# krishnanlab/PecanPy

Hardware: AMD Instinct MI355X
Metric: million walk-steps/sec on RMAT-22 SparseOTF p=0.5 q=2 (higher is better)
Workload: dtype f32

## Files before the change

include/pecanpy_amd.h:

```cpp
#ifndef PECANPY_AMD_H
#define PECANPY_AMD_H

#include <stdint.h>

#ifdef __cplusplus
extern "C" {
#endif

typedef struct pw_graph pw_graph;

typedef enum {
    PW_OK = 0,
    PW_ERR_INVALID = -1,
    PW_ERR_HIP = -2,
    PW_ERR_NO_DEVICE = -3,
    PW_ERR_UNSUPPORTED = -4,
    PW_ERR_NOMEM = -5
} pw_status;

typedef enum {
    PW_MODE_SPARSE_OTF = 0,
    PW_MODE_DENSE_OTF = 1,
    PW_MODE_PRECOMP = 2,
    PW_MODE_FIRST_ORDER_UNWEIGHTED = 3,
// ... 281 lines not shown
int pw_selftest_seqscan_f64(const double *x, uint32_t n, double r, int use_target, uint32_t chunk,
                            uint32_t *index, double *sum);

int pw_selftest_exact_decision(const uint8_t *cls, uint32_t n, float w_out, float w_prev, const double *r,
                               uint32_t n_r, uint32_t *chain, uint32_t *exact);
int pw_selftest_lane(int on_device, int device, const uint8_t *cls, uint32_t n, float w_out, float w_prev, const double *r,
                     uint32_t n_r, uint32_t *chain, uint32_t *lane, uint32_t *kmax, uint32_t *tight, uint32_t *chain_lane);
int pw_selftest_lane_floats(int on_device, int device, const uint8_t *cls, uint32_t n, float w_out, float w_prev,
                            const double *r, uint32_t n_r, uint32_t *chain, uint32_t *lane, float *tots);
int pw_selftest_lane_unit_bounded(const uint8_t *cls, uint32_t n, float w_out, float w_prev, const double *r, uint32_t n_r,
                                  uint32_t *chain, uint32_t *lane);
int pw_selftest_lane_unit_tight(const uint8_t *cls, uint32_t n, float w_out, float w_prev, const double *r, uint32_t n_r,
                                uint32_t *chain, uint32_t *lane, uint32_t *tight);
int pw_selftest_lane_weighted(const float *vals, const float *base, const uint8_t *cls, uint32_t n, const double *r,
                              uint32_t n_r, uint32_t *chain, uint32_t *lane);
int pw_selftest_exact_decision_f64(const uint8_t *cls, uint32_t n, double w_out, double w_prev, const double *r,
                                   uint32_t n_r, uint32_t *chain, uint32_t *exact);

#ifdef __cplusplus
}
#endif
#endif
```

pecanpy_amd/_lib.py:

```python
import ctypes as C
import os
import subprocess

_HERE = os.path.dirname(os.path.abspath(__file__))
LIB_PATH = os.environ.get("PECANPY_AMD_LIB") or os.path.join(_HERE, "libpecanpy_amd.so")
_lib = None


class PwStats(C.Structure):
    _fields_ = [
        ("total_steps", C.c_uint64),
        ("overflow_reads", C.c_uint64),
        ("clamped_reads", C.c_uint64),
        ("dead_end_walks", C.c_uint64),
        ("repair_rounds", C.c_uint64),
        ("walk_kernel_ms", C.c_double),
        ("rng_kernel_ms", C.c_double),
        ("walk_kernel_launches", C.c_uint32),
        ("stream_addressing", C.c_uint32),
        ("lane_kernel", C.c_uint32),
        ("lane_rounds", C.c_uint32),
        ("redo_walks", C.c_uint64),
        ("list_entries_read", C.c_uint64),
        ("ambiguous_steps", C.c_uint64),
# ... 310 lines not shown
    "pw_corpus_dev_shape": (C.c_int, [C.c_void_p] + [C.POINTER(C.c_uint64)] * 3),
    "pw_corpus_dev_fill": (C.c_int, [C.c_void_p, C.c_void_p]),
    "pw_corpus_dev_export": (C.c_int, [C.c_void_p, C.c_void_p]),
    "pw_corpus_dev_destroy": (None, [C.c_void_p]),
    "pw_selftest_edgelist_weight": (C.c_int, [C.c_char_p, C.c_uint64, _f64p]),
    "pw_selftest_edgelist_line": (C.c_int, [C.c_char_p, C.c_uint64, C.c_uint64, C.c_char_p, C.c_int, _u32p, C.c_void_p, _f64p]),
    "pw_selftest_exact_decision": (C.c_int, [C.c_void_p, C.c_uint32, C.c_float, C.c_float, C.c_void_p, C.c_uint32,
                                             C.c_void_p, C.c_void_p]),
    "pw_selftest_lane": (C.c_int, [C.c_int, C.c_int, C.c_void_p, C.c_uint32, C.c_float, C.c_float, C.c_void_p, C.c_uint32,
                                   C.c_void_p, C.c_void_p, C.c_void_p, C.c_void_p, C.c_void_p]),
    "pw_selftest_lane_floats": (C.c_int, [C.c_int, C.c_int, C.c_void_p, C.c_uint32, C.c_float, C.c_float, C.c_void_p, C.c_uint32,
                                          C.c_void_p, C.c_void_p, C.c_void_p]),
    "pw_selftest_lane_unit_bounded": (C.c_int, [C.c_void_p, C.c_uint32, C.c_float, C.c_float, C.c_void_p, C.c_uint32, C.c_void_p, C.c_void_p]),
    "pw_selftest_lane_unit_tight": (C.c_int, [C.c_void_p, C.c_uint32, C.c_float, C.c_float, C.c_void_p, C.c_uint32, C.c_void_p, C.c_void_p, C.c_void_p]),
    "pw_selftest_lane_weighted": (C.c_int, [C.c_void_p, C.c_void_p, C.c_void_p, C.c_uint32, C.c_void_p, C.c_uint32, C.c_void_p, C.c_void_p]),
    "pw_selftest_exact_decision_f64": (C.c_int, [C.c_void_p, C.c_uint32, C.c_double, C.c_double, C.c_void_p,
                                                 C.c_uint32, C.c_void_p, C.c_void_p]),
    "pw_selftest_seqscan_f32": (C.c_int, [C.c_void_p, C.c_uint32, C.c_double, C.c_int, C.c_uint32,
                                          _u32p, _f32p]),
    "pw_selftest_seqscan_f64": (C.c_int, [C.c_void_p, C.c_uint32, C.c_double, C.c_int, C.c_uint32,
                                          _u32p, _f64p]),
}


class PwError(RuntimeError):
    pass


def build(verbose=False):
    cmd = ["make", "-C", os.path.join(_HERE, "csrc")]
# ... 66 lines not shown
```

pecanpy_amd/csrc/pecanpy_amd.hip:

```cpp
#include <hip/hip_runtime.h>
#include <stdio.h>
#include <unistd.h>
#include <stdlib.h>
#include <string.h>

#include <new>
#include <random>
#include <algorithm>
#include <cerrno>
#include <chrono>
#include <condition_variable>
#include <functional>
#include <future>
#include <memory>
#include <mutex>
#include <cmath>
#include <string>
#include <thread>
#include <vector>

#include "../../include/pecanpy_amd.h"
#include "aux_kernels.hip.h"
#include "devmem.hpp"
#include "edgelist.hpp"
// ... 5030 lines not shown
        uint32_t kc = n;
        for (uint32_t k = 0; k < n; k++) {
            c = c + x[cls[k]];
            if (c >= r[i]) { kc = k; break; }
        }
        chain[i] = kc;
        const pw::ExactThresholds64 th = pw::exact_thresholds_f64(r[i] * S, (double)n, wmax);
        const uint32_t k1 = (uint32_t)(std::lower_bound(E.begin(), E.end(), th.lo) - E.begin());
        exact[i] = (k1 < n && E[k1] >= th.hi) ? k1 : 0xffffffffu;
    }
    return PW_OK;
}

namespace {

struct LaneRow {
    std::vector<uint16_t> cl16;
    std::vector<uint32_t> cl32;
    uint32_t n_cl = 0, pp = 0xffffffffu, wide = 0;
    uint32_t piv_off = 0;
    float tot = 0, x_in = 0, x_out = 0, x_prev = 0;
    pw::ListView view() const { return pw::list_view_of(wide ? (const void *)cl32.data() : (const void *)cl16.data(), wide, n_cl, piv_off); }
};

int lane_row_setup(const uint8_t *cls, uint32_t n, float w_out, float w_prev, LaneRow &row, bool need_pow2 = true) {
    auto pow2 = [](float w) { int e = 0; return std::frexp(w, &e) == 0.5f; };
    if (need_pow2 && (!pow2(w_out) || !pow2(w_prev))) return fail(PW_ERR_UNSUPPORTED, "biases must be powers of two");
    if (!(w_out > 0.0f) || !(w_prev > 0.0f)) return fail(PW_ERR_INVALID, "biases must be positive");
    uint32_t cnt[3] = {0, 0, 0};
    row.wide = n > 65536u ? 1u : 0u;
    for (uint32_t k = 0; k < n; k++) {
        if (cls[k] > 2) return fail(PW_ERR_INVALID, "class must be 0 (out), 1 (common) or 2 (prev)");
        cnt[cls[k]]++;
        if (cls[k] == 1) { if (row.wide) row.cl32.push_back(k); else row.cl16.push_back((uint16_t)k); }
        if (cls[k] == 2) row.pp = k;
    }
    if (cnt[2] > 1) return fail(PW_ERR_INVALID, "at most one prev");
    row.n_cl = cnt[1];
    row.cl16.resize(row.cl16.size() + 8, 0xffffu);
    row.cl32.resize(row.cl32.size() + 8, 0xffffffffu);
    if (pw::list_has_pivots(row.wide, row.n_cl) && !getenv("PW_SELFTEST_NO_PIVOTS")) {
        const uint32_t np = pw::list_pivot_count(row.wide), step = pw::list_pivot_step(row.wide, row.n_cl);
        row.piv_off = (uint32_t)(row.wide ? row.cl32.size() : row.cl16.size());
        for (uint32_t k = 0; k < np; k++) {
            if (row.wide) row.cl32.push_back(row.cl32[(size_t)(k + 1) * step]);
            else row.cl16.push_back(row.cl16[(size_t)(k + 1) * step]);
        }
    }
    row.tot = (float)((double)cnt[1] + (double)cnt[0] * (double)w_out + (double)cnt[2] * (double)w_prev);
    row.x_in = 1.0f / row.tot;
    row.x_out = row.x_in * w_out;
    row.x_prev = row.x_in * w_prev;
    return 0;
}

}

namespace pw {
PW_HD void lane_selftest_one(uint32_t n, const ListView &cl, uint32_t n_cl, uint32_t pp, float w_out, float w_prev, double r,
                             uint32_t *out) {
    LaneStep ls{0.0f, 0u, 0u, 0u, 0u, 0u, 0u};
    const uint32_t lane = lane_decide(n, n_cl, pp, r, w_out, w_prev, cl, ls);
// ... 277 lines not shown
            if (vals[k] < base[k]) any_neg = true;
            drun += (double)vals[k] - (double)base[k];
            dl.push_back(drun);
            if (wide) cl32.push_back(k); else cl16.push_back((uint16_t)k);
        } else if (cls[k] == 2) {
            if (pp != 0xffffffffu) return fail(PW_ERR_INVALID, "at most one prev");
            pp = k;
            dprev = (double)vals[k] - (double)base[k];
        } else if (cls[k] != 0 || vals[k] != base[k]) return fail(PW_ERR_INVALID, "class 0 elements carry their base value");
    }
    const uint32_t n_cl = (uint32_t)dl.size();
    cl16.resize(cl16.size() + 8, 0xffffu);
    cl32.resize(cl32.size() + 8, 0xffffffffu);
    uint32_t piv_off = 0;
    if (pw::list_has_pivots(wide, n_cl)) {
        const uint32_t np = pw::list_pivot_count(wide), step = pw::list_pivot_step(wide, n_cl);
        piv_off = (uint32_t)(wide ? cl32.size() : cl16.size());
        for (uint32_t k = 0; k < np; k++) { if (wide) cl32.push_back(cl32[(size_t)(k + 1) * step]); else cl16.push_back(cl16[(size_t)(k + 1) * step]); }
    }
    dl.push_back(0.0);
    const pw::ListView view = pw::list_view_of(wide ? (const void *)cl32.data() : (const void *)cl16.data(), wide, n_cl, piv_off);
    if (any_pos && any_neg) return fail(PW_ERR_INVALID, "the common neighbours' differences must share one sign (that of q - 1)");
    const pw::WeightedRow wr{pq.data(), dl.data(), dprev, !any_neg};
    for (uint32_t i = 0; i < n_r; i++) {
        uint32_t lo = 0, hi = n;
        while (lo < hi) { const uint32_t mid = (lo + hi) >> 1; if ((double)c[mid] >= r[i]) hi = mid; else lo = mid + 1; }
        chain[i] = lo;
        uint32_t probes = 0, k_safe = 0;
        lane[i] = pw::lane_decide_weighted(n, n_cl, pp, r[i], tot, wr, view, probes, k_safe);
        if (k_safe > chain[i]) return fail(PW_ERR_INVALID, "lane_decide_weighted: k_safe beyond the chain's position");
    }
    return PW_OK;
}

PW_EXPORT int pw_noise_thresholds_csr(const uint32_t *indptr, const float *data, uint32_t n_nodes, double gamma, float *thr) {
    if (!indptr || !thr || (!data && indptr[n_nodes] != 0)) return fail(PW_ERR_INVALID, "null pointer");
    pw::noise_thresholds_csr(indptr, data, n_nodes, gamma, thr);
    return PW_OK;
}

PW_EXPORT int pw_noise_thresholds_csr_numpy1(const uint32_t *indptr, const float *data, uint32_t n_nodes, double gamma, float *thr) {
    if (!indptr || !thr || (!data && indptr[n_nodes] != 0)) return fail(PW_ERR_INVALID, "null pointer");
    pw::noise_thresholds_csr(indptr, data, n_nodes, gamma, thr, true);
    return PW_OK;
}

PW_EXPORT int pw_noise_thresholds_csr_f64(const uint32_t *indptr, const float *data, uint32_t n_nodes, double gamma, float *thr) {
    if (!indptr || !thr) return fail(PW_ERR_INVALID, "null pointer");
    pw::noise_thresholds_csr_f64(indptr, data, n_nodes, gamma, thr);
// ... 76 lines not shown
```

pecanpy_amd/csrc/seqscan.h:

```cpp
#pragma once
#include <math.h>
#include <stdint.h>
#include <string.h>

#if defined(__HIPCC__)
#define PW_HD __host__ __device__ __forceinline__
#define PW_HD_CALL __host__ __device__ __attribute__((noinline))
#else
#define PW_HD inline
#define PW_HD_CALL inline
#endif

namespace pw {

template <typename T> struct FloatTraits;

template <> struct FloatTraits<float> {
    using UInt = uint32_t;
    static constexpr int MANT = 23;
    static constexpr int EXP_MASK = 0xff;
    static PW_HD UInt bits(float x) {
#if defined(__HIP_DEVICE_COMPILE__)
        return __float_as_uint(x);
#else
// ... 159 lines not shown
    if (prev_pos != 0xffffffffu && prev_pos >= s && k >= prev_pos) {
        const uint32_t need2 = need > wp ? need - wp : 0u;
        k = s + ((need2 + wo_m1) >> sh_out);
        if (k < prev_pos) k = prev_pos;
        e_k = base + ((k - s) << sh_out) + wp;
    }
    return k;
}

struct ListWin {
    uint32_t v[4];
};
constexpr uint32_t LIST_PIVOTS_NARROW = 20, LIST_PIVOTS_WIDE = 10;
PW_HD uint32_t list_pivot_count(uint32_t wide) { return wide ? LIST_PIVOTS_WIDE : LIST_PIVOTS_NARROW; }
PW_HD bool list_has_pivots(uint32_t wide, uint32_t n) { return n > list_pivot_count(wide); }
PW_HD uint32_t list_pivot_step(uint32_t wide, uint32_t n) { return wide ? n / (LIST_PIVOTS_WIDE + 1u) : n / (LIST_PIVOTS_NARROW + 1u); }

struct ListView {
    const void *p;
    uint32_t wide;
    const void *piv = nullptr;
    uint32_t npiv = 0;
    uint32_t step = 0;
    uint32_t tail = 0xffffffffu;
    uint32_t inl = 0;
    uint32_t tshift = 10;
#if defined(__HIP_DEVICE_COMPILE__)
    __device__ __forceinline__ uint32_t tail_entry(uint32_t i) const {
        const uint32_t o = 8u + (wide ? i << 2 : i << 1);
        const uint32_t addr = tail + ((o >> 4) << tshift) + (o & 15u);
        return wide ? *(const __attribute__((address_space(3))) uint32_t *)(uintptr_t)addr
                    : (uint32_t) * (const __attribute__((address_space(3))) uint16_t *)(uintptr_t)addr;
    }
#endif
    PW_HD uint32_t at(uint32_t i) const {
#if defined(__HIP_DEVICE_COMPILE__)
        if (tail != 0xffffffffu && inl) return tail_entry(i);
#endif
// ... 19 lines not shown
        }
#endif
        if (wide) {
            struct __attribute__((packed, aligned(4))) Raw { uint32_t v[4]; };
            const Raw raw = *(const Raw *)((const uint32_t *)p + w0);
            w.v[0] = raw.v[0]; w.v[1] = raw.v[1]; w.v[2] = raw.v[2]; w.v[3] = raw.v[3];
        } else {
            struct __attribute__((aligned(8))) Raw2 { uint32_t x, y; };
            const Raw2 raw = *(const Raw2 *)((const uint16_t *)p + w0);
            w.v[0] = raw.x & 0xffffu; w.v[1] = raw.x >> 16; w.v[2] = raw.y & 0xffffu; w.v[3] = raw.y >> 16;
        }
        return w;
    }
};

PW_HD ListView list_view_of(const void *cl, uint32_t wide, uint32_t n_cl, uint32_t piv_off) {
    ListView v{cl, wide};
    if (piv_off && list_has_pivots(wide, n_cl)) {
        v.piv = wide ? (const void *)((const uint32_t *)cl + piv_off) : (const void *)((const uint16_t *)cl + piv_off);
        v.npiv = list_pivot_count(wide);
        v.step = list_pivot_step(wide, n_cl);
    }
    return v;
}

PW_HD uint32_t list_lower_bound_pos(const ListView &cl, uint32_t n, uint32_t x) {
    uint32_t lo = 0, hi = n;
    if (cl.npiv) {
        uint32_t klo = 0, khi = cl.npiv;
        while (klo < khi) {
            const uint32_t km = (klo + khi) >> 1;
            if (cl.pivot(km) >= x) { khi = km; hi = (km + 1u) * cl.step; }
            else { klo = km + 1u; lo = (km + 1u) * cl.step + 1u; }
        }
    }
    while (lo < hi) {
        const uint32_t mid = (lo + hi) >> 1;
        if (cl.at(mid) < x) lo = mid + 1u; else hi = mid;
    }
    return lo;
}

PW_HD uint64_t div_floor_small(uint64_t a, uint64_t b) {
    uint64_t q = (uint64_t)((double)a / (double)b);
    if (q * b > a) q--;
    else if ((q + 1u) * b <= a) q++;
    return q;
}

struct SearchResult {
    uint32_t f;
    uint32_t p_below, p_at;
    uint64_t v_below, v_at;
    bool has_below;
};
template <class Eval>
PW_HD void list_search_pivots(const ListView &cl, const Eval &ev, uint64_t target, uint32_t &lo, uint32_t &hi, SearchResult &r) {
    uint32_t klo = 0, khi = cl.npiv;
    while (klo < khi) {
        const uint32_t km = (klo + khi) >> 1;
        const uint32_t ik = (km + 1u) * cl.step;
        if (ik < lo) { klo = km + 1u; continue; }
        const uint32_t P = cl.pivot(km);
        const uint64_t v = ev(ik, P);
        if (v >= target) { khi = km; hi = ik; r.p_at = P; r.v_at = v; }
        else { klo = km + 1u; lo = ik + 1u; r.p_below = P; r.v_below = v; r.has_below = true; }
    }
}

template <class Eval>
PW_HD SearchResult list_search(const ListView &cl, uint32_t lo_min, uint32_t n, const Eval &ev, uint64_t target, uint32_t &reads) {
    SearchResult r;
    r.p_below = 0; r.v_below = 0; r.has_below = false; r.p_at = 0xffffffffu; r.v_at = 0;
    uint32_t lo = lo_min, hi = n;
    if (cl.npiv) list_search_pivots(cl, ev, target, lo, hi, r);
    while (lo < hi) {
        const uint32_t mid = (lo + hi) >> 1;
        const uint32_t P = cl.at(mid);
        reads++;
        const uint64_t v = ev(mid, P);
        if (v >= target) { hi = mid; r.p_at = P; r.v_at = v; }
        else { lo = mid + 1u; r.p_below = P; r.v_below = v; r.has_below = true; }
    }
    r.f = lo;
    return r;
}

template <class Eval>
PW_HD SearchResult list_search_wide(const ListView &cl, uint32_t lo_min, uint32_t n, const Eval &ev, uint64_t target, uint32_t &reads) {
    SearchResult r;
    r.p_below = 0; r.v_below = 0; r.has_below = false; r.p_at = 0xffffffffu; r.v_at = 0;
    uint32_t lo = lo_min, hi = n;
    while (hi - lo >= 3u && hi > lo) {
        const uint32_t m2 = lo + ((hi - lo) >> 1);
        const uint32_t m1 = lo + ((m2 - lo) >> 1);
        const uint32_t m3 = m2 + 1u + ((hi - m2 - 1u) >> 1);
        const uint32_t P1 = cl.at(m1), P2 = cl.at(m2), P3 = cl.at(m3);
// ... 667 lines not shown
```

pecanpy_amd/csrc/walk_lanes.hip.h:

```cpp
#pragma once
#include "scan.hip.h"
#include "walk_sparse.hip.h"

namespace pw {

struct SuspRec {
    uint32_t job, j, s0, d;
    uint32_t n_in, pp, e, coff;
    uint32_t kmax, choice, soff_lo, soff_hi;
    float tot, wo;
    double r;
};
static_assert(sizeof(SuspRec) == 64, "queue record is four 16-byte accesses");

struct VerRec {
    uint32_t kmax, n_in, pp, choice;
    uint32_t e, coff, d, job;
    float tot, wo;
    double r;
};
static_assert(sizeof(VerRec) == 48, "verification record is three 16-byte stores");

constexpr uint32_t LANE_NEEDS_WAVE = 0xfffffff9u;
constexpr uint32_t LANE_EAGER_MARK = 0xffffffffu;
// ... 775 lines not shown
        } else {
            DecideCtx dc;
            SearchResult sr;
            sr.f = 0; sr.p_below = 0; sr.v_below = 0; sr.has_below = false; sr.p_at = 0xffffffffu; sr.v_at = 0;
            uint32_t s_lo = 0, s_hi = 0;
            bool need = false, go = false;
            const bool narrow = A.d <= 65536u;
            if (runnable && !nolist) {
                wo = A.j >= 2 ? w_out : 1.0f;
                choice = lane_decide_begin(A.d, A.n_in, A.pp, r, wo, w_prev, ls, dc);
                go = choice != LANE_REDO;
                if (go && A.n_in) {
                    const MassEval ev64{A.pp, dc.sh_in, dc.sh_out, dc.sh_prev};
                    const uint32_t wide = narrow ? 0u : 1u;
                    const bool inl = narrow && A.n_in <= EL_INLINE;
                    const uint32_t step = inl ? 1u : list_pivot_step(wide, A.n_in);
                    uint32_t klo = 0, khi = inl ? A.n_in : (list_has_pivots(wide, A.n_in) ? list_pivot_count(wide) : 0u);
                    s_hi = A.n_in;
                    while (klo < khi) {
                        const uint32_t km = (klo + khi) >> 1;
                        const uint32_t ik = inl ? km : (km + 1u) * step;
                        const uint32_t P = narrow ? q_u16(24u + (km << 1)) : q_u32(24u + (km << 2));
                        const uint32_t vm = (uint32_t)ev64(ik, P);
                        if (vm >= dc.lo_th) { khi = km; s_hi = ik; sr.p_at = P; sr.v_at = vm; }
                        else { klo = km + 1u; s_lo = ik + 1u; sr.p_below = P; sr.v_below = vm; sr.has_below = true; }
                    }
                    need = !inl && s_lo < s_hi;
                    sr.f = s_lo;
                }
            }
            for (uint32_t trip = 0; ballot(need); trip++) {
                const uint32_t esh = narrow ? 1u : 2u;
                const uint64_t lbase = (uint64_t)A.coff * 16u;
                uint32_t g = s_lo + ((s_hi - s_lo) >> 1);
                if (need && trip < 2u && sr.has_below && sr.p_at != 0xffffffffu && sr.v_at > sr.v_below) {
                    const float t = (float)(dc.lo_th - (uint32_t)sr.v_below) / (float)((uint32_t)sr.v_at - (uint32_t)sr.v_below);
                    const float fe = (float)s_lo - 1.0f + t * (float)(s_hi - s_lo + 1u);
                    const uint32_t gi = fe > 0.0f ? (uint32_t)fe : 0u;
                    g = gi < s_lo ? s_lo : (gi >= s_hi ? s_hi - 1u : gi);
                }
                const uint32_t sec = (uint32_t)((lbase + ((uint64_t)g << esh)) >> 6);
                quad_fetch(need, a.clist, sec);
                if (need) {
                    const MassEval ev64{A.pp, dc.sh_in, dc.sh_out, dc.sh_prev};
                    auto ev = [&](uint32_t i, uint32_t P) -> uint32_t { return (uint32_t)ev64(i, P); };
                    const uint64_t sb = (uint64_t)sec << 6;
                    const uint32_t w_lo = sb > lbase ? (uint32_t)((sb - lbase) >> esh) : 0u;
                    uint32_t w_hi = (uint32_t)((sb + 64u - lbase) >> esh);
                    if (w_hi > A.n_in) w_hi = A.n_in;
                    const uint32_t c_lo = w_lo > s_lo ? w_lo : s_lo, c_hi = w_hi < s_hi ? w_hi : s_hi;
                    const uint32_t eoff = (uint32_t)(lbase - sb);
                    auto ent = [&](uint32_t i) -> uint32_t { const uint32_t o = eoff + (i << esh); return narrow ? q_u16(o) : q_u32(o); };
                    const uint32_t P0 = ent(c_lo);
                    const uint32_t v0 = ev(c_lo, P0);
                    if (v0 >= dc.lo_th) { s_hi = c_lo; sr.p_at = P0; sr.v_at = v0; }
                    else {
                        sr.p_below = P0; sr.v_below = v0; sr.has_below = true;
                        s_lo = c_lo + 1u;
                        if (s_lo < c_hi) {
                            const uint32_t P1 = ent(c_hi - 1u);
                            const uint32_t v1 = ev(c_hi - 1u, P1);
                            if (v1 < dc.lo_th) { s_lo = c_hi; sr.p_below = P1; sr.v_below = v1; }
                            else {
                                uint32_t l2 = s_lo, h2 = c_hi - 1u;
                                sr.p_at = P1; sr.v_at = v1;
                                while (l2 < h2) {
                                    const uint32_t mid = (l2 + h2) >> 1;
                                    const uint32_t P = ent(mid);
                                    const uint32_t vm = ev(mid, P);
                                    if (vm >= dc.lo_th) { h2 = mid; sr.p_at = P; sr.v_at = vm; }
                                    else { l2 = mid + 1u; sr.p_below = P; sr.v_below = vm; }
                                }
                                s_lo = s_hi = l2;
                            }
                        }
                    }
                    ls.probes += 32u;
                    sr.f = s_lo;
                    need = s_lo < s_hi;
                }
            }
            if (go) choice = lane_decide_end(A.d, A.n_in, A.pp, dc, &sr, ls);
            n_probes += ls.probes;
        }
        if (nolist && !WEIGHTED) {
            wo = w_out;
            ls.kmax = LANE_EAGER_MARK;
            if (INPLACE && !a.susp) choice = LANE_NEEDS_WAVE;
        }
#ifdef PW_PROF_LANES
        {
// ... 780 lines not shown
    const uint32_t d_h = indptr[h + 1] - indptr[h];
    const bool mine = rev == NOT_FOUND || d_h > d_k || (d_h == d_k && h > k);
    return (mine && d_h >= 2u && d_k) ? log_pair_slots(d_h, d_k) : 0u;
}
struct LogSlots {
    const ELine *lines;
    const uint32_t *indptr, *edge_row;
    __device__ uint32_t operator()(uint64_t e2) const { return log_slots(lines, indptr, edge_row, e2); }
};

__global__ void __launch_bounds__(256)
lane_scatter_kernel(LaneBuildArgs a, const uint32_t *__restrict__ edge_row, const uint32_t *__restrict__ vm0, uint32_t nnz) {
    const int lane = lane_id();
    const uint64_t e2 = (uint64_t)blockIdx.x * 256 + threadIdx.x;
    bool todo = false;
    uint32_t n = 0, nseg = 1, segbase = 0, s_k = 0, rev = NOT_FOUND, k_wide = 0, h_wide = 0;
    uint8_t *p2 = nullptr, *p1 = nullptr;
    const uint32_t *src = nullptr;
    if (e2 < nnz && log_slots(a.lines, a.indptr, edge_row, e2)) {
        const uint4 r0 = *(const uint4 *)(a.lines + e2);
        const uint2 r1 = *((const uint2 *)(a.lines + e2) + 2);
        const uint32_t h = edge_row[e2], d_k = r0.w;
        const uint32_t s_h = a.indptr[h], d_h = a.indptr[h + 1] - s_h;
        n = r0.y; rev = r0.z; s_k = r1.x;
        k_wide = list_is_narrow(d_k) ? 0u : 1u;
        h_wide = log_wide(d_h) ? 1u : 0u;
        nseg = d_h > (uint32_t)LB_SEG ? (d_h + LB_SEG - 1) / LB_SEG : 1u;
        todo = n != 0u && !(nseg == 1u && list_is_inline(d_k, n)) && n <= a.max_len;
        if (todo) {
            p2 = (uint8_t *)list_base(a.lines, a.clist, (uint32_t)e2, d_k, n, r1.y);
            if (rev != NOT_FOUND) {
                const uint32_t e1 = s_k + rev;
                p1 = (uint8_t *)list_base(a.lines, a.clist, e1, d_h, a.lines[e1].n_in, a.lines[e1].coff);
            }
            src = a.log + a.log_off[e2];
            if (nseg > 1u) segbase = vm0[h] + ((uint32_t)e2 - s_h) * nseg;
        }
    }
    auto put = [](uint8_t *q2, uint8_t *q1, uint32_t at, uint32_t pk, uint32_t ph, uint32_t kw, uint32_t hw) {
        if (kw) ((uint32_t *)q2)[at] = pk; else ((uint16_t *)q2)[at] = (uint16_t)pk;
        if (q1) { if (hw) ((uint32_t *)q1)[at] = ph; else ((uint16_t *)q1)[at] = (uint16_t)ph; }
    };
    const bool small_one = todo && nseg == 1u && n <= 32u;
    if (small_one) {
        for (uint32_t i = 0; i < n; i++) {
            const uint32_t v = src[i];
            put(p2, p1, i, rev == NOT_FOUND ? v : (v & 0xffffu), v >> 16, k_wide, 0u);
        }
        if (list_has_pivots(k_wide, n)) {
            const uint32_t np = list_pivot_count(k_wide), step = list_pivot_step(k_wide, n);
            uint8_t *dst = (uint8_t *)(a.lines + e2) + 24;
            for (uint32_t t = 0; t < np; t++) {
                const uint32_t v = src[(t + 1u) * step];
                put(dst, nullptr, t, rev == NOT_FOUND ? v : (v & 0xffffu), 0u, k_wide, 0u);
            }
        }
        if (p1 && list_has_pivots(0u, n)) {
            const uint32_t step = list_pivot_step(0u, n);
            uint16_t *dst = (uint16_t *)((uint8_t *)(a.lines + (s_k + rev)) + 24);
            for (uint32_t t = 0; t < LIST_PIVOTS_NARROW; t++) dst[t] = (uint16_t)(src[(t + 1u) * step] >> 16);
        }
    }
    uint64_t big = ballot(todo && !small_one);
    while (big) {
        const int l = __ffsll((long long)big) - 1;
        big &= big - 1ull;
        const uint32_t nsg = readlane_u32(nseg, l), sb = readlane_u32(segbase, l), nn = readlane_u32(n, l);
        const uint32_t kw = readlane_u32(k_wide, l), hw = readlane_u32(h_wide, l), norev = readlane_u32(rev, l) == NOT_FOUND ? 1u : 0u;
        const uint32_t *sp = (const uint32_t *)readlane_u64((uint64_t)src, l);
        uint8_t *q2 = (uint8_t *)readlane_u64((uint64_t)p2, l), *q1 = (uint8_t *)readlane_u64((uint64_t)p1, l);
        uint32_t out = 0;
        for (uint32_t sg = 0; sg < nsg; sg++) {
            const uint32_t cnt = nsg > 1u ? a.segcnt[sb + sg] : nn;
            const uint32_t lo = nsg > 1u ? a.seglo[sb + sg] : 0u;
            for (uint32_t i = (uint32_t)lane; i < cnt; i += WAVE) {
// ... 1 lines not shown
                    const unsigned long long v = ((const unsigned long long *)sp)[lo + i];
                    put(q2, q1, out + i, (uint32_t)v, (uint32_t)(v >> 32), kw, 1u);
                } else {
                    const uint32_t v = sp[lo + i];
                    put(q2, q1, out + i, norev ? v : (v & 0xffffu), v >> 16, kw, 0u);
                }
            }
            out += cnt;
        }
        const uint32_t e2l = (uint32_t)((uint64_t)blockIdx.x * 256 + (threadIdx.x & ~63u) + (uint32_t)l);
        const uint32_t s_kl = readlane_u32(s_k, l), revl = readlane_u32(rev, l);
        for (int which = 0; which < 2; which++) {
            const uint32_t wide = which == 0 ? kw : hw;
            if (which == 1 && !q1) break;
            if (!list_has_pivots(wide, nn)) continue;
            const uint32_t np = list_pivot_count(wide), step = list_pivot_step(wide, nn);
            if ((uint32_t)lane < np) {
                uint32_t target = ((uint32_t)lane + 1u) * step, base = 0, pk = 0, ph = 0;
                for (uint32_t sg = 0; sg < nsg; sg++) {
                    const uint32_t cnt = nsg > 1u ? a.segcnt[sb + sg] : nn;
                    if (target < base + cnt) {
                        const uint32_t lo = nsg > 1u ? a.seglo[sb + sg] : 0u;
                        if (hw) { const unsigned long long v = ((const unsigned long long *)sp)[lo + target - base]; pk = (uint32_t)v; ph = (uint32_t)(v >> 32); }
                        else { const uint32_t v = sp[lo + target - base]; pk = norev ? v : (v & 0xffffu); ph = v >> 16; }
                        break;
                    }
                    base += cnt;
                }
                uint8_t *dst = (uint8_t *)(a.lines + (which == 0 ? e2l : s_kl + revl)) + 24;
                if (wide) ((uint32_t *)dst)[lane] = which == 0 ? pk : ph; else ((uint16_t *)dst)[lane] = (uint16_t)(which == 0 ? pk : ph);
            }
        }
    }
}

__global__ void __launch_bounds__(256)
self_loop_bits_kernel(const uint32_t *__restrict__ indptr, const uint32_t *__restrict__ indices, uint32_t n_nodes, uint32_t *bits) {
    const uint32_t v = blockIdx.x * blockDim.x + threadIdx.x;
    if (v >= n_nodes) return;
    const uint32_t s0 = indptr[v], d = indptr[v + 1] - s0;
    const uint32_t i = lower_bound_u32(indices + s0, d, v);
    if (i < d && indices[s0 + i] == v) atomicOr(bits + (v >> 5), 1u << (v & 31u));
}
__global__ void __launch_bounds__(256)
// ... 44 lines not shown
    if (!u) return;
    const uint32_t n = lines[e].n_in;
    atomicAdd(hist + (n < hist_len ? n : hist_len - 1u), (unsigned long long)u);
}

__global__ void __launch_bounds__(256)
eline_pivots_kernel(ELine *lines, const uint8_t *__restrict__ clist, uint32_t n_lines, uint32_t first = 0) {
    const uint64_t e = (uint64_t)first + (uint64_t)blockIdx.x * blockDim.x + threadIdx.x;
    if (e >= n_lines) return;
    const uint4 r0 = *(const uint4 *)(lines + e);
    if (r0.x == NOT_FOUND) return;
    const uint32_t n_in = r0.y, d = r0.w;
    if (list_is_inline(d, n_in) || lines[e].coff == EL_NO_LIST) return;
    const uint32_t wide = list_is_narrow(d) ? 0u : 1u;
    if (!list_has_pivots(wide, n_in)) return;
    const uint32_t np = list_pivot_count(wide), step = list_pivot_step(wide, n_in);
    const uint8_t *p = clist + (uint64_t)lines[e].coff * 16u;
    uint8_t *dst = (uint8_t *)(lines + e) + 24;
    for (uint32_t k = 0; k < np; k++) {
        const uint32_t idx = (k + 1u) * step;
        if (wide) ((uint32_t *)dst)[k] = ((const uint32_t *)p)[idx];
        else ((uint16_t *)dst)[k] = ((const uint16_t *)p)[idx];
    }
}

struct ListUnits {
    const ELine *lines;
    uint32_t max_len;
    __device__ uint32_t operator()(uint64_t e) const { return list_units(lines, e, max_len); }
};
struct ListOffset {
    ELine *lines;
    uint32_t max_len;
    __device__ void operator()(uint64_t e, uint64_t units_before) const {
        const uint4 r0 = *(const uint4 *)(lines + e);
        lines[e].coff = (!list_is_inline(r0.w, r0.y) && r0.y > max_len) ? EL_NO_LIST : (uint32_t)units_before;
    }
// ... 64 lines not shown
```

pecanpy_amd/csrc/walk_sparse.hip.h:

```cpp
#pragma once
#include "counters.h"
#include "seqscan.h"
#include "wave.h"

namespace pw {

constexpr uint32_t NOT_FOUND = 0xffffffffu;

struct ELine {
    uint32_t nxt;
    uint32_t n_in;
    uint32_t rev_pos;
    uint32_t deg;
    uint32_t s0;
    uint32_t coff;
    uint16_t inl[20];
};
static_assert(sizeof(ELine) == 64, "edge line is one 64-byte sector");
constexpr uint32_t EL_INLINE = 20;
constexpr uint32_t EL_NO_LIST = 0xffffffffu;
__device__ __forceinline__ bool edge_list_stored(uint32_t d, uint32_t n_in, uint32_t coff) {
    return (d <= 65536u && n_in <= EL_INLINE) || coff != EL_NO_LIST;
}

__device__ __forceinline__ ListView edge_list(const ELine *lines, const uint8_t *clist, uint32_t e, uint32_t d, uint32_t n_in,
                                              uint32_t coff) {
    const bool narrow = d <= 65536u;
    const bool inl = narrow && n_in <= EL_INLINE;
    const uint8_t *p = inl ? (const uint8_t *)(lines + e) + 24 : clist + (uint64_t)coff * 16u;
    ListView v{p, narrow ? 0u : 1u};
    if (!inl && list_has_pivots(v.wide, n_in)) {
        v.piv = (const uint8_t *)(lines + e) + 24;
        v.npiv = list_pivot_count(v.wide);
        v.step = list_pivot_step(v.wide, n_in);
    }
    return v;
}

struct CsrDev {
    const uint32_t *__restrict__ indptr;
    const uint32_t *__restrict__ indices;
    const void *__restrict__ data;
    const float *__restrict__ thr;
    const uint64_t *__restrict__ adjbits;
    uint32_t words_per_row;
    const uint32_t *__restrict__ foff;
    const uint64_t *__restrict__ fbits;
    const uint2 *__restrict__ kf;
    const uint64_t *__restrict__ tab_off;
    const uint64_t *__restrict__ slots;
// ... 1450 lines not shown
```

Before: 15800.

## Align list pivots to 64-byte sector boundaries with power-of-two spacing

```diff
diff --git a/include/pecanpy_amd.h b/include/pecanpy_amd.h
--- a/include/pecanpy_amd.h
+++ b/include/pecanpy_amd.h
@@ -319,6 +319,9 @@
                                 uint32_t *chain, uint32_t *lane, uint32_t *tight);
 int pw_selftest_lane_weighted(const float *vals, const float *base, const uint8_t *cls, uint32_t n, const double *r,
                               uint32_t n_r, uint32_t *chain, uint32_t *lane);
+int pw_selftest_pivot_layout(uint32_t wide, uint32_t n, uint32_t coff, uint32_t *out);
+int pw_selftest_pivot_search(const uint32_t *list, uint32_t n, uint32_t wide, uint32_t coff, const uint32_t *targets,
+                             uint32_t n_t, uint32_t *piv, uint32_t *sec, uint32_t *sectors);
 int pw_selftest_exact_decision_f64(const uint8_t *cls, uint32_t n, double w_out, double w_prev, const double *r,
                                    uint32_t n_r, uint32_t *chain, uint32_t *exact);
 
diff --git a/pecanpy_amd/_lib.py b/pecanpy_amd/_lib.py
--- a/pecanpy_amd/_lib.py
+++ b/pecanpy_amd/_lib.py
@@ -348,6 +348,9 @@
     "pw_selftest_lane_unit_bounded": (C.c_int, [C.c_void_p, C.c_uint32, C.c_float, C.c_float, C.c_void_p, C.c_uint32, C.c_void_p, C.c_void_p]),
     "pw_selftest_lane_unit_tight": (C.c_int, [C.c_void_p, C.c_uint32, C.c_float, C.c_float, C.c_void_p, C.c_uint32, C.c_void_p, C.c_void_p, C.c_void_p]),
     "pw_selftest_lane_weighted": (C.c_int, [C.c_void_p, C.c_void_p, C.c_void_p, C.c_uint32, C.c_void_p, C.c_uint32, C.c_void_p, C.c_void_p]),
+    "pw_selftest_pivot_layout": (C.c_int, [C.c_uint32, C.c_uint32, C.c_uint32, C.c_void_p]),
+    "pw_selftest_pivot_search": (C.c_int, [C.c_void_p, C.c_uint32, C.c_uint32, C.c_uint32, C.c_void_p, C.c_uint32,
+                                          C.c_void_p, C.c_void_p, C.c_void_p]),
     "pw_selftest_exact_decision_f64": (C.c_int, [C.c_void_p, C.c_uint32, C.c_double, C.c_double, C.c_void_p,
                                                  C.c_uint32, C.c_void_p, C.c_void_p]),
     "pw_selftest_seqscan_f32": (C.c_int, [C.c_void_p, C.c_uint32, C.c_double, C.c_int, C.c_uint32,
diff --git a/pecanpy_amd/csrc/pecanpy_amd.hip b/pecanpy_amd/csrc/pecanpy_amd.hip
--- a/pecanpy_amd/csrc/pecanpy_amd.hip
+++ b/pecanpy_amd/csrc/pecanpy_amd.hip
@@ -5068,6 +5068,14 @@
 
 namespace {
 
+template <typename E>
+uint32_t append_pivots(std::vector<E> &v, uint32_t wide, uint32_t n_cl, uint32_t coff) {
+    const pw::PivotLayout pl = pw::list_pivot_layout(wide, n_cl, coff);
+    const uint32_t off = (uint32_t)v.size();
+    for (uint32_t k = 0; k < pw::list_pivot_count(wide); k++) v.push_back(k < pl.npiv ? v[(size_t)pl.first + (size_t)k * pl.step] : (E)~(E)0);
+    return off;
+}
+
 struct LaneRow {
     std::vector<uint16_t> cl16;
     std::vector<uint32_t> cl32;
@@ -5094,12 +5102,7 @@
     row.cl16.resize(row.cl16.size() + 8, 0xffffu);
     row.cl32.resize(row.cl32.size() + 8, 0xffffffffu);
     if (pw::list_has_pivots(row.wide, row.n_cl) && !getenv("PW_SELFTEST_NO_PIVOTS")) {
-        const uint32_t np = pw::list_pivot_count(row.wide), step = pw::list_pivot_step(row.wide, row.n_cl);
-        row.piv_off = (uint32_t)(row.wide ? row.cl32.size() : row.cl16.size());
-        for (uint32_t k = 0; k < np; k++) {
-            if (row.wide) row.cl32.push_back(row.cl32[(size_t)(k + 1) * step]);
-            else row.cl16.push_back(row.cl16[(size_t)(k + 1) * step]);
-        }
+        row.piv_off = row.wide ? append_pivots(row.cl32, 1u, row.n_cl, 0u) : append_pivots(row.cl16, 0u, row.n_cl, 0u);
     }
     row.tot = (float)((double)cnt[1] + (double)cnt[0] * (double)w_out + (double)cnt[2] * (double)w_prev);
     row.x_in = 1.0f / row.tot;
@@ -5407,9 +5410,7 @@
     cl32.resize(cl32.size() + 8, 0xffffffffu);
     uint32_t piv_off = 0;
     if (pw::list_has_pivots(wide, n_cl)) {
-        const uint32_t np = pw::list_pivot_count(wide), step = pw::list_pivot_step(wide, n_cl);
-        piv_off = (uint32_t)(wide ? cl32.size() : cl16.size());
-        for (uint32_t k = 0; k < np; k++) { if (wide) cl32.push_back(cl32[(size_t)(k + 1) * step]); else cl16.push_back(cl16[(size_t)(k + 1) * step]); }
+        piv_off = wide ? append_pivots(cl32, 1u, n_cl, 0u) : append_pivots(cl16, 0u, n_cl, 0u);
     }
     dl.push_back(0.0);
     const pw::ListView view = pw::list_view_of(wide ? (const void *)cl32.data() : (const void *)cl16.data(), wide, n_cl, piv_off);
@@ -5426,6 +5427,41 @@
     return PW_OK;
 }
 
+PW_EXPORT int pw_selftest_pivot_layout(uint32_t wide, uint32_t n, uint32_t coff, uint32_t *out) {
+    if (!out || wide > 1u || !pw::list_has_pivots(wide, n)) return fail(PW_ERR_INVALID, "pw_selftest_pivot_layout: the list has no pivots");
+    const pw::PivotLayout pl = pw::list_pivot_layout(wide, n, coff);
+    out[0] = pl.npiv; out[1] = pl.first; out[2] = pl.step;
+    return PW_OK;
+}
+PW_EXPORT int pw_selftest_pivot_search(const uint32_t *list, uint32_t n, uint32_t wide, uint32_t coff, const uint32_t *targets, uint32_t n_t,
+                                       uint32_t *piv, uint32_t *sec, uint32_t *sectors) {
+    if (!list || !targets || !piv || !sec || !sectors || wide > 1u || !pw::list_has_pivots(wide, n))
+        return fail(PW_ERR_INVALID, "pw_selftest_pivot_search: bad argument");
+    std::vector<uint16_t> cl16;
+    std::vector<uint32_t> cl32;
+    for (uint32_t i = 0; i < n; i++) {
+        if (i && list[i] <= list[i - 1]) return fail(PW_ERR_INVALID, "pw_selftest_pivot_search: the list must ascend");
+        if (wide) cl32.push_back(list[i]);
+        else if (list[i] > 0xffffu) return fail(PW_ERR_INVALID, "pw_selftest_pivot_search: a narrow entry above 65535");
+        else cl16.push_back((uint16_t)list[i]);
+    }
+    const uint32_t piv_off = wide ? append_pivots(cl32, 1u, n, coff) : append_pivots(cl16, 0u, n, coff);
+    const pw::ListView view = pw::list_view_of(wide ? (const void *)cl32.data() : (const void *)cl16.data(), wide, n, piv_off, coff);
+    auto ev = [](uint32_t, uint32_t P) -> uint64_t { return (uint64_t)P; };
+    for (uint32_t t = 0; t < n_t; t++) {
+        uint32_t reads = 0;
+        const pw::SearchResult a = pw::list_search(view, 0u, n, ev, (uint64_t)targets[t], reads);
+        piv[t] = a.f;
+        sectors[t] = 0;
+        const pw::SearchResult b = pw::list_search_sectors(view, n, coff, ev, targets[t], sectors[t]);
+        sec[t] = b.f;
+        if (a.has_below != b.has_below || (a.has_below && (a.p_below != b.p_below || a.v_below != b.v_below)) || a.p_at != b.p_at ||
+            (a.p_at != 0xffffffffu && a.v_at != b.v_at))
+            return fail(PW_ERR_INVALID, "pw_selftest_pivot_search: the two searches disagree about the entries around the answer");
+    }
+    return PW_OK;
+}
+
 PW_EXPORT int pw_noise_thresholds_csr(const uint32_t *indptr, const float *data, uint32_t n_nodes, double gamma, float *thr) {
     if (!indptr || !thr || (!data && indptr[n_nodes] != 0)) return fail(PW_ERR_INVALID, "null pointer");
     pw::noise_thresholds_csr(indptr, data, n_nodes, gamma, thr);
diff --git a/pecanpy_amd/csrc/seqscan.h b/pecanpy_amd/csrc/seqscan.h
--- a/pecanpy_amd/csrc/seqscan.h
+++ b/pecanpy_amd/csrc/seqscan.h
@@ -197,7 +197,25 @@
 constexpr uint32_t LIST_PIVOTS_NARROW = 20, LIST_PIVOTS_WIDE = 10;
 PW_HD uint32_t list_pivot_count(uint32_t wide) { return wide ? LIST_PIVOTS_WIDE : LIST_PIVOTS_NARROW; }
 PW_HD bool list_has_pivots(uint32_t wide, uint32_t n) { return n > list_pivot_count(wide); }
-PW_HD uint32_t list_pivot_step(uint32_t wide, uint32_t n) { return wide ? n / (LIST_PIVOTS_WIDE + 1u) : n / (LIST_PIVOTS_NARROW + 1u); }
+constexpr uint32_t LIST_SECTOR_SHIFT_NARROW = 5, LIST_SECTOR_SHIFT_WIDE = 4;
+PW_HD uint32_t list_sector_shift(uint32_t wide) { return wide ? LIST_SECTOR_SHIFT_WIDE : LIST_SECTOR_SHIFT_NARROW; }
+PW_HD uint32_t list_sector_phase(uint32_t wide, uint32_t coff) { return (coff & 3u) << (wide ? 2u : 3u); }
+struct PivotLayout {
+    uint32_t npiv, first, step;
+};
+PW_HD PivotLayout list_pivot_layout(uint32_t wide, uint32_t n, uint32_t coff) {
+    const uint32_t a = list_sector_phase(wide, coff), m = n - 1u;
+    const uint32_t t = wide ? m / LIST_PIVOTS_WIDE : m / LIST_PIVOTS_NARROW;
+    uint32_t lg = 32u - (uint32_t)__builtin_clz(t);
+    const uint32_t c1 = ((a + m) >> (lg - 1u)) - (a >> (lg - 1u));
+    if (c1 <= list_pivot_count(wide)) lg--;
+    const uint32_t q0 = a >> lg;
+    PivotLayout L;
+    L.npiv = ((a + m) >> lg) - q0;
+    L.first = ((q0 + 1u) << lg) - a;
+    L.step = 1u << lg;
+    return L;
+}
 
 struct ListView {
     const void *p;
@@ -205,6 +223,8 @@
     const void *piv = nullptr;
     uint32_t npiv = 0;
     uint32_t step = 0;
+    uint32_t first = 0;
+    PW_HD uint32_t pivot_index(uint32_t k) const { return first + k * step; }
     uint32_t tail = 0xffffffffu;
     uint32_t inl = 0;
     uint32_t tshift = 10;
@@ -254,13 +274,17 @@
     }
 };
 
-PW_HD ListView list_view_of(const void *cl, uint32_t wide, uint32_t n_cl, uint32_t piv_off) {
+PW_HD void list_view_set_pivots(ListView &v, const void *piv, uint32_t n, uint32_t coff) {
+    const PivotLayout L = list_pivot_layout(v.wide, n, coff);
+    v.piv = piv;
+    v.npiv = L.npiv;
+    v.step = L.step;
+    v.first = L.first;
+}
+PW_HD ListView list_view_of(const void *cl, uint32_t wide, uint32_t n_cl, uint32_t piv_off, uint32_t coff = 0) {
     ListView v{cl, wide};
-    if (piv_off && list_has_pivots(wide, n_cl)) {
-        v.piv = wide ? (const void *)((const uint32_t *)cl + piv_off) : (const void *)((const uint16_t *)cl + piv_off);
-        v.npiv = list_pivot_count(wide);
-        v.step = list_pivot_step(wide, n_cl);
-    }
+    if (piv_off && list_has_pivots(wide, n_cl))
+        list_view_set_pivots(v, wide ? (const void *)((const uint32_t *)cl + piv_off) : (const void *)((const uint16_t *)cl + piv_off), n_cl, coff);
     return v;
 }
 
@@ -270,8 +294,8 @@
         uint32_t klo = 0, khi = cl.npiv;
         while (klo < khi) {
             const uint32_t km = (klo + khi) >> 1;
-            if (cl.pivot(km) >= x) { khi = km; hi = (km + 1u) * cl.step; }
-            else { klo = km + 1u; lo = (km + 1u) * cl.step + 1u; }
+            if (cl.pivot(km) >= x) { khi = km; hi = cl.pivot_index(km); }
+            else { klo = km + 1u; lo = cl.pivot_index(km) + 1u; }
         }
     }
     while (lo < hi) {
@@ -299,7 +323,7 @@
     uint32_t klo = 0, khi = cl.npiv;
     while (klo < khi) {
         const uint32_t km = (klo + khi) >> 1;
-        const uint32_t ik = (km + 1u) * cl.step;
+        const uint32_t ik = cl.pivot_index(km);
         if (ik < lo) { klo = km + 1u; continue; }
         const uint32_t P = cl.pivot(km);
         const uint64_t v = ev(ik, P);
@@ -321,6 +345,54 @@
         const uint64_t v = ev(mid, P);
         if (v >= target) { hi = mid; r.p_at = P; r.v_at = v; }
         else { lo = mid + 1u; r.p_below = P; r.v_below = v; r.has_below = true; }
+    }
+    r.f = lo;
+    return r;
+}
+
+PW_HD bool sector_range_is_one(uint32_t a, uint32_t ssh, uint32_t s_lo, uint32_t s_hi) {
+    return ((a + s_lo) >> ssh) == ((a + s_hi - 1u) >> ssh);
+}
+PW_HD uint32_t sector_guess_entry(uint32_t s_lo, uint32_t s_hi, uint32_t trip, const SearchResult &sr, uint32_t target) {
+    uint32_t g = s_lo + ((s_hi - s_lo) >> 1);
+    if (trip < 2u && sr.has_below && sr.p_at != 0xffffffffu && sr.v_at > sr.v_below) {
+        const float t = (float)(target - (uint32_t)sr.v_below) / (float)((uint32_t)sr.v_at - (uint32_t)sr.v_below);
+        const float fe = (float)s_lo - 1.0f + t * (float)(s_hi - s_lo + 1u);
+        const uint32_t gi = fe > 0.0f ? (uint32_t)fe : 0u;
+        g = gi < s_lo ? s_lo : (gi >= s_hi ? s_hi - 1u : gi);
+    }
+    return g;
+}
+template <class Ent, class Eval>
+PW_HD void sector_settle(uint32_t a, uint32_t ssh, uint32_t n, uint32_t sec, const Ent &ent, const Eval &ev, uint32_t target,
+                         uint32_t &s_lo, uint32_t &s_hi, SearchResult &sr) {
+    const uint32_t b0 = sec << ssh;
+    const uint32_t w_lo = b0 > a ? b0 - a : 0u;
+    uint32_t w_hi = b0 + (1u << ssh) - a;
+    if (w_hi > n) w_hi = n;
+    const uint32_t c_lo = w_lo > s_lo ? w_lo : s_lo, c_hi = w_hi < s_hi ? w_hi : s_hi;
+    uint32_t l2 = c_lo, h2 = c_hi;
+    while (l2 < h2) {
+        const uint32_t mid = (l2 + h2) >> 1;
+        const uint32_t P = ent(mid);
+        const uint32_t vm = (uint32_t)ev(mid, P);
+        if (vm >= target) { h2 = mid; sr.p_at = P; sr.v_at = vm; }
+        else { l2 = mid + 1u; sr.p_below = P; sr.v_below = vm; sr.has_below = true; }
+    }
+    if (l2 == c_hi) s_lo = c_hi;
+    else { s_hi = l2; if (l2 > c_lo) s_lo = l2; }
+}
+template <class Eval>
+PW_HD SearchResult list_search_sectors(const ListView &cl, uint32_t n, uint32_t coff, const Eval &ev, uint32_t target, uint32_t &sectors) {
+    SearchResult r;
+    r.p_below = 0; r.v_below = 0; r.has_below = false; r.p_at = 0xffffffffu; r.v_at = 0;
+    uint32_t lo = 0, hi = n;
+    if (cl.npiv) list_search_pivots(cl, ev, (uint64_t)target, lo, hi, r);
+    const uint32_t a = list_sector_phase(cl.wide, coff), ssh = list_sector_shift(cl.wide);
+    for (uint32_t trip = 0; lo < hi; trip++) {
+        const uint32_t g = sector_range_is_one(a, ssh, lo, hi) ? lo : sector_guess_entry(lo, hi, trip, r, target);
+        sectors++;
+        sector_settle(a, ssh, n, (a + g) >> ssh, [&](uint32_t i) { return cl.at(i); }, ev, target, lo, hi, r);
     }
     r.f = lo;
     return r;
diff --git a/pecanpy_amd/csrc/walk_lanes.hip.h b/pecanpy_amd/csrc/walk_lanes.hip.h
--- a/pecanpy_amd/csrc/walk_lanes.hip.h
+++ b/pecanpy_amd/csrc/walk_lanes.hip.h
@@ -813,12 +813,16 @@
                     const MassEval ev64{A.pp, dc.sh_in, dc.sh_out, dc.sh_prev};
                     const uint32_t wide = narrow ? 0u : 1u;
                     const bool inl = narrow && A.n_in <= EL_INLINE;
-                    const uint32_t step = inl ? 1u : list_pivot_step(wide, A.n_in);
-                    uint32_t klo = 0, khi = inl ? A.n_in : (list_has_pivots(wide, A.n_in) ? list_pivot_count(wide) : 0u);
+                    PivotLayout pl{A.n_in, 0u, 1u};
+                    if (!inl) {
+                        if (list_has_pivots(wide, A.n_in)) pl = list_pivot_layout(wide, A.n_in, A.coff);
+                        else pl.npiv = 0u;
+                    }
+                    uint32_t klo = 0, khi = pl.npiv;
                     s_hi = A.n_in;
                     while (klo < khi) {
                         const uint32_t km = (klo + khi) >> 1;
-                        const uint32_t ik = inl ? km : (km + 1u) * step;
+                        const uint32_t ik = pl.first + km * pl.step;
                         const uint32_t P = narrow ? q_u16(24u + (km << 1)) : q_u32(24u + (km << 2));
                         const uint32_t vm = (uint32_t)ev64(ik, P);
                         if (vm >= dc.lo_th) { khi = km; s_hi = ik; sr.p_at = P; sr.v_at = vm; }
@@ -829,51 +833,17 @@
                 }
             }
             for (uint32_t trip = 0; ballot(need); trip++) {
-                const uint32_t esh = narrow ? 1u : 2u;
-                const uint64_t lbase = (uint64_t)A.coff * 16u;
-                uint32_t g = s_lo + ((s_hi - s_lo) >> 1);
-                if (need && trip < 2u && sr.has_below && sr.p_at != 0xffffffffu && sr.v_at > sr.v_below) {
-                    const float t = (float)(dc.lo_th - (uint32_t)sr.v_below) / (float)((uint32_t)sr.v_at - (uint32_t)sr.v_below);
-                    const float fe = (float)s_lo - 1.0f + t * (float)(s_hi - s_lo + 1u);
-                    const uint32_t gi = fe > 0.0f ? (uint32_t)fe : 0u;
-                    g = gi < s_lo ? s_lo : (gi >= s_hi ? s_hi - 1u : gi);
-                }
-                const uint32_t sec = (uint32_t)((lbase + ((uint64_t)g << esh)) >> 6);
-                quad_fetch(need, a.clist, sec);
+                const uint32_t wide = narrow ? 0u : 1u, esh = narrow ? 1u : 2u;
+                const uint32_t ssh = list_sector_shift(wide), ph = list_sector_phase(wide, A.coff);
+                uint32_t g = s_lo;
+                if (need && !sector_range_is_one(ph, ssh, s_lo, s_hi)) g = sector_guess_entry(s_lo, s_hi, trip, sr, dc.lo_th);
+                const uint32_t rel = (ph + g) >> ssh;
+                quad_fetch(need, a.clist, (A.coff >> 2) + rel);
                 if (need) {
                     const MassEval ev64{A.pp, dc.sh_in, dc.sh_out, dc.sh_prev};
-                    auto ev = [&](uint32_t i, uint32_t P) -> uint32_t { return (uint32_t)ev64(i, P); };
-                    const uint64_t sb = (uint64_t)sec << 6;
-                    const uint32_t w_lo = sb > lbase ? (uint32_t)((sb - lbase) >> esh) : 0u;
-                    uint32_t w_hi = (uint32_t)((sb + 64u - lbase) >> esh);
-                    if (w_hi > A.n_in) w_hi = A.n_in;
-                    const uint32_t c_lo = w_lo > s_lo ? w_lo : s_lo, c_hi = w_hi < s_hi ? w_hi : s_hi;
-                    const uint32_t eoff = (uint32_t)(lbase - sb);
-                    auto ent = [&](uint32_t i) -> uint32_t { const uint32_t o = eoff + (i << esh); return narrow ? q_u16(o) : q_u32(o); };
-                    const uint32_t P0 = ent(c_lo);
-                    const uint32_t v0 = ev(c_lo, P0);
-                    if (v0 >= dc.lo_th) { s_hi = c_lo; sr.p_at = P0; sr.v_at = v0; }
-                    else {
-                        sr.p_below = P0; sr.v_below = v0; sr.has_below = true;
-                        s_lo = c_lo + 1u;
-                        if (s_lo < c_hi) {
-                            const uint32_t P1 = ent(c_hi - 1u);
-                            const uint32_t v1 = ev(c_hi - 1u, P1);
-                            if (v1 < dc.lo_th) { s_lo = c_hi; sr.p_below = P1; sr.v_below = v1; }
-                            else {
-                                uint32_t l2 = s_lo, h2 = c_hi - 1u;
-                                sr.p_at = P1; sr.v_at = v1;
-                                while (l2 < h2) {
-                                    const uint32_t mid = (l2 + h2) >> 1;
-                                    const uint32_t P = ent(mid);
-                                    const uint32_t vm = ev(mid, P);
-                                    if (vm >= dc.lo_th) { h2 = mid; sr.p_at = P; sr.v_at = vm; }
-                                    else { l2 = mid + 1u; sr.p_below = P; sr.v_below = vm; }
-                                }
-                                s_lo = s_hi = l2;
-                            }
-                        }
-                    }
+                    const uint32_t eoff = ph - (rel << ssh);
+                    auto ent = [&](uint32_t i) -> uint32_t { const uint32_t o = (eoff + i) << esh; return narrow ? q_u16(o) : q_u32(o); };
+                    sector_settle(ph, ssh, A.n_in, rel, ent, ev64, dc.lo_th, s_lo, s_hi, sr);
                     ls.probes += 32u;
                     sr.f = s_lo;
                     need = s_lo < s_hi;
@@ -1684,7 +1654,7 @@
     const int lane = lane_id();
     const uint64_t e2 = (uint64_t)blockIdx.x * 256 + threadIdx.x;
     bool todo = false;
-    uint32_t n = 0, nseg = 1, segbase = 0, s_k = 0, rev = NOT_FOUND, k_wide = 0, h_wide = 0;
+    uint32_t n = 0, nseg = 1, segbase = 0, s_k = 0, rev = NOT_FOUND, k_wide = 0, h_wide = 0, coff2 = 0;
     uint8_t *p2 = nullptr, *p1 = nullptr;
     const uint32_t *src = nullptr;
     if (e2 < nnz && log_slots(a.lines, a.indptr, edge_row, e2)) {
@@ -1692,7 +1662,7 @@
         const uint2 r1 = *((const uint2 *)(a.lines + e2) + 2);
         const uint32_t h = edge_row[e2], d_k = r0.w;
         const uint32_t s_h = a.indptr[h], d_h = a.indptr[h + 1] - s_h;
-        n = r0.y; rev = r0.z; s_k = r1.x;
+        n = r0.y; rev = r0.z; s_k = r1.x; coff2 = r1.y;
         k_wide = list_is_narrow(d_k) ? 0u : 1u;
         h_wide = log_wide(d_h) ? 1u : 0u;
         nseg = d_h > (uint32_t)LB_SEG ? (d_h + LB_SEG - 1) / LB_SEG : 1u;
@@ -1718,17 +1688,18 @@
             put(p2, p1, i, rev == NOT_FOUND ? v : (v & 0xffffu), v >> 16, k_wide, 0u);
         }
         if (list_has_pivots(k_wide, n)) {
-            const uint32_t np = list_pivot_count(k_wide), step = list_pivot_step(k_wide, n);
+            const uint32_t np = list_pivot_count(k_wide);
+            const PivotLayout pl = list_pivot_layout(k_wide, n, coff2);
             uint8_t *dst = (uint8_t *)(a.lines + e2) + 24;
             for (uint32_t t = 0; t < np; t++) {
-                const uint32_t v = src[(t + 1u) * step];
-                put(dst, nullptr, t, rev == NOT_FOUND ? v : (v & 0xffffu), 0u, k_wide, 0u);
+                const uint32_t v = t < pl.npiv ? src[pl.first + t * pl.step] : 0xffffffffu;
+                put(dst, nullptr, t, (rev == NOT_FOUND || t >= pl.npiv) ? v : (v & 0xffffu), 0u, k_wide, 0u);
             }
         }
         if (p1 && list_has_pivots(0u, n)) {
-            const uint32_t step = list_pivot_step(0u, n);
+            const PivotLayout pl = list_pivot_layout(0u, n, a.lines[s_k + rev].coff);
             uint16_t *dst = (uint16_t *)((uint8_t *)(a.lines + (s_k + rev)) + 24);
-            for (uint32_t t = 0; t < LIST_PIVOTS_NARROW; t++) dst[t] = (uint16_t)(src[(t + 1u) * step] >> 16);
+            for (uint32_t t = 0; t < LIST_PIVOTS_NARROW; t++) dst[t] = t < pl.npiv ? (uint16_t)(src[pl.first + t * pl.step] >> 16) : (uint16_t)0xffffu;
         }
     }
     uint64_t big = ballot(todo && !small_one);
@@ -1760,10 +1731,12 @@
             const uint32_t wide = which == 0 ? kw : hw;
             if (which == 1 && !q1) break;
             if (!list_has_pivots(wide, nn)) continue;
-            const uint32_t np = list_pivot_count(wide), step = list_pivot_step(wide, nn);
+            const uint32_t np = list_pivot_count(wide);
+            const uint32_t line = which == 0 ? e2l : s_kl + revl;
+            const PivotLayout pl = list_pivot_layout(wide, nn, a.lines[line].coff);
             if ((uint32_t)lane < np) {
-                uint32_t target = ((uint32_t)lane + 1u) * step, base = 0, pk = 0, ph = 0;
-                for (uint32_t sg = 0; sg < nsg; sg++) {
+                uint32_t target = pl.first + (uint32_t)lane * pl.step, base = 0, pk = 0xffffffffu, ph = 0xffffffffu;
+                for (uint32_t sg = 0; (uint32_t)lane < pl.npiv && sg < nsg; sg++) {
                     const uint32_t cnt = nsg > 1u ? a.segcnt[sb + sg] : nn;
                     if (target < base + cnt) {
                         const uint32_t lo = nsg > 1u ? a.seglo[sb + sg] : 0u;
@@ -1773,7 +1746,7 @@
                     }
                     base += cnt;
                 }
-                uint8_t *dst = (uint8_t *)(a.lines + (which == 0 ? e2l : s_kl + revl)) + 24;
+                uint8_t *dst = (uint8_t *)(a.lines + line) + 24;
                 if (wide) ((uint32_t *)dst)[lane] = which == 0 ? pk : ph; else ((uint16_t *)dst)[lane] = (uint16_t)(which == 0 ? pk : ph);
             }
         }
@@ -1848,13 +1821,14 @@
     if (list_is_inline(d, n_in) || lines[e].coff == EL_NO_LIST) return;
     const uint32_t wide = list_is_narrow(d) ? 0u : 1u;
     if (!list_has_pivots(wide, n_in)) return;
-    const uint32_t np = list_pivot_count(wide), step = list_pivot_step(wide, n_in);
-    const uint8_t *p = clist + (uint64_t)lines[e].coff * 16u;
+    const uint32_t np = list_pivot_count(wide), coff = lines[e].coff;
+    const PivotLayout pl = list_pivot_layout(wide, n_in, coff);
+    const uint8_t *p = clist + (uint64_t)coff * 16u;
     uint8_t *dst = (uint8_t *)(lines + e) + 24;
     for (uint32_t k = 0; k < np; k++) {
-        const uint32_t idx = (k + 1u) * step;
-        if (wide) ((uint32_t *)dst)[k] = ((const uint32_t *)p)[idx];
-        else ((uint16_t *)dst)[k] = ((const uint16_t *)p)[idx];
+        const uint32_t idx = pl.first + k * pl.step;
+        if (wide) ((uint32_t *)dst)[k] = k < pl.npiv ? ((const uint32_t *)p)[idx] : 0xffffffffu;
+        else ((uint16_t *)dst)[k] = k < pl.npiv ? ((const uint16_t *)p)[idx] : (uint16_t)0xffffu;
     }
 }
 
diff --git a/pecanpy_amd/csrc/walk_sparse.hip.h b/pecanpy_amd/csrc/walk_sparse.hip.h
--- a/pecanpy_amd/csrc/walk_sparse.hip.h
+++ b/pecanpy_amd/csrc/walk_sparse.hip.h
@@ -29,11 +29,7 @@
     const bool inl = narrow && n_in <= EL_INLINE;
     const uint8_t *p = inl ? (const uint8_t *)(lines + e) + 24 : clist + (uint64_t)coff * 16u;
     ListView v{p, narrow ? 0u : 1u};
-    if (!inl && list_has_pivots(v.wide, n_in)) {
-        v.piv = (const uint8_t *)(lines + e) + 24;
-        v.npiv = list_pivot_count(v.wide);
-        v.step = list_pivot_step(v.wide, n_in);
-    }
+    if (!inl && list_has_pivots(v.wide, n_in)) list_view_set_pivots(v, (const uint8_t *)(lines + e) + 24, n_in, coff);
     return v;
 }
 
```

After: 15900 (median of 6 runs). No clear change (+0.6%).
